# johannes-graeter/limo

Measured on AMD Instinct MI355X. Metric: keyframe-BA window solves/sec (5 KF, ~2k landmarks), higher is better.
Workload: dtype f64; 1 GPU; C2: KITTI-00-shaped windows, 5 keyframes x 2000 landmarks, LiDAR depth + ground plane, solveTrimmed schedule {2, trim 5%, <=100 LM iterations}; batch_windows_per_gpu=16384, distinct_windows_per_gpu=4096, observations_per_batch=144288124, depth_observations_per_batch=68405568, parallelism=single, converged=16328

## Files before the change

### limo_amd/csrc/kba_items.hpp

```cpp
#pragma once
#include "kba_layout.hpp"
#include "kba_lm.hpp"
#include "kba_math.hpp"

#ifndef KBA_SYNC
#define KBA_SYNC() ((void)0)
#endif
#if defined(KBA_PROFILE_TICKS) && defined(__HIPCC__)
__device__ long long kba_ticks[2][24];
#endif
#if defined(KBA_PROFILE_TICKS) && defined(__HIP_DEVICE_COMPILE__)
#define KBA_TICK(n)                                                                   \
    do {                                                                              \
        if (w == 0 && (tid == 0 || tid == nt - 1)) kba_ticks[tid != 0][n] = clock64(); \
    } while (0)
#else
#define KBA_TICK(n) ((void)0)
#endif

namespace kba {

struct LinLane {
    double e[kLinPartial];
    int fail;
// ... 310 lines not shown
    const WinDesc& wd = bv.win[w];
    part[0] = part[1] = part[5] = 0.0;
    for (int j = 0; j < wd.n_view; ++j) {
        cam[j].fail = 0;
        for (int i = 0; i < kLinPartial; ++i) cam[j].e[i] = 0.0;
    }
    const int state = bv.lm_state[gl];
    if (state == 0) return 0;
    LmAcc acc;
    for (int i = 0; i < 6; ++i) acc.V[i] = 0.0;
    for (int i = 0; i < 3; ++i) acc.g[i] = 0.0;
    int fail = 0;
    for (int j = 0; j < wd.n_view; ++j) {
        const int s = bv.lm_slot[(int64_t)j * bv.SL + gl];
        if (s < 0) continue;
        LinIn in;
        lin_fetch(bv, s, gl, in);
        const double* vl = bv.view_lin + (int64_t)kViewLin * (wd.view0 + j);
        double r3[3], c4[4];
        if (j < wd.n_view_fixed0) {
            if (!lin_obs<false>(vl, c, in, want_cost, r3, c4, cam[j])) fail = 1;
        } else {
            if (!lin_obs<true>(vl, c, in, want_cost, r3, c4, cam[j])) fail = 1;
        }
        bv.obs_c[s] = c4[0];
        bv.obs_c[bv.SO + s] = c4[3];
        lin_lm_accum(vl, r3, c4, acc);
    }
    if (state == 1) {
        LmTailIn t;
        lin_lm_tail_fetch(bv, w, gl, t);
        lin_lm_finish(bv, c, gl, bv.lm + 3 * (int64_t)gl, t, acc, part);
    }
    return fail;
}

KBA_HD void trim_residual_lane(const BatchView& bv, int b, int t, double* plane_rep, double* plane_dep) {
    if (t >= bv.blk_n[b]) return;
    const int view = bv.blk_view[b];
    const int64_t o = bv.blk_obs0[b] + t;
    const int gl = bv.obs_lm[o];
    double nr = -1.0, nd = -1.0;
    if (bv.lm_state[gl]) {
        const double* cam = bv.view_cam + 16 * (int64_t)view;
        double ruv[2], rd, zc[3];
        if (obs_residual(bv.pose + 7 * (int64_t)bv.view_kf[view], cam + 4, cam + 13, cam[0], cam[1], cam[2],
                         bv.lm + 3 * (int64_t)gl, bv.obs_u[o], bv.obs_v[o], bv.obs_d[o], ruv, &rd, zc)) {
            nr = sqrt(ruv[0] * ruv[0] + ruv[1] * ruv[1]);
        } else {
// ... 178 lines not shown
    while ((ca + 1) * lda - (ca + 1) * ca / 2 <= i) ++ca;
    cb = ca + (i - (ca * lda - ca * (ca - 1) / 2));
}
KBA_HD int schur_col(int i, int nfq);
KBA_HD int64_t schur_need_offset(int ca, int cb, int nf, int nfq, int nfp) {
    if (cb < nf) return (int64_t)schur_col(ca, nfq) * nfp + schur_col(cb, nfq);
    const int za = schur_col(ca, nfq);
    return za < nfq ? (int64_t)za * nfp + nfq : (int64_t)nfq * nfp + za;
}
KBA_HD void slab_reduce_entry(const BatchView& bv, int w, int n_shards, int i) {
    const WinDesc& wd = bv.win[w];
    const int64_t slab = (int64_t)wd.nf_pad * wd.nf_pad;
    int ca, cb;
    schur_need_decode(i, wd.nf, ca, cb);
    const double* sp = bv.S_part + wd.spart_off + schur_need_offset(ca, cb, wd.nf, wd.nfq, wd.nf_pad);
    double a = 0.0;
    const int q0 = (ca >= wd.nfq || (cb >= wd.nfq && cb < wd.nf)) ? wd.n_sblk_plain : 0;
    for (int q = q0; q < wd.n_sblk; ++q) a += sp[q * slab];
    bv.S_red[wd.sred_off / n_shards + i] = a;
}

KBA_HD int schur_col(int i, int nfq) {
    return i + (i >= nfq ? 1 : 0);
}

struct LogProd {
    double m;
    int e;
};
KBA_HD void logprod_mul(LogProd& a, double x) {
    int ex;
    a.m *= frexp(x, &ex);
    a.e += ex;
}
KBA_HD double logprod_log(const LogProd& a) { return log(a.m) + static_cast<double>(a.e) * 0.69314718055994530942; }

KBA_HD void backsub_lane(const BatchView& bv, const SolveConsts& c, int w, int gl, double* part) {
    part[2] = part[3] = part[4] = part[6] = part[7] = 0.0;
    const int state = bv.lm_state[gl];
    const double* xp = bv.lm + 3 * (int64_t)gl;
    const double x[3] = {xp[0], xp[1], xp[2]};
    double xc[3] = {x[0], x[1], x[2]};
    if (state == 0) {
        double* o = bv.lm_c + 3 * (int64_t)gl;
        o[0] = xc[0];
        o[1] = xc[1];
// ... 671 lines not shown
    const int nc = wd.nc, nf = wd.nf, nfp = wd.nf_pad, lda = nf + 1;
    double* A = scratch;
    double* y = A + nf * lda;
    double* dl = y + nf;
    int* fl = reinterpret_cast<int*>(dl + nc);
    double* red = dl + nc + (nf + 1) / 2 + 1;
    double* Hs = red + coop_red_doubles(3, nt);
    const double radius = bv.st[w].radius;
    const double* Hg = bv.Hcc + wd.hcc_off;
    const double* sc = bv.scale_c + wd.cam0;
    const int32_t* cs = bv.cslot + wd.cam0;
    double* yc = bv.yc + wd.cam0;
    double* dc = bv.delta_c + wd.cam0;
    const int slab = c.schur_packed ? schur_need_pad(nf) : nfp * nfp;
    const int nfq = wd.nfq;
    KBA_TICK(8);
    for (int a = tid; a < nc; a += nt)
        if (cs[a] >= 0) fl[cs[a]] = a;
    KBA_SYNC();
    const double* sp = c.schur_nslab > 0 ? bv.S_red + wd.sred_off : bv.S_part + wd.spart_off;
    const int n_need = nf * (nf + 1) / 2 + nf;
    const int n_slab = c.schur_nslab > 0 ? c.schur_nslab : schur_slabs(wd, c.schur_span, c.schur_span_gp);
    const int q_gp = c.schur_nslab > 0 ? 0 : (schur_plain_slabs(wd, c.schur_span) & ~3);
    constexpr int kE = 4;
    for (int i0 = tid; i0 < n_need; i0 += kE * nt) {
        double s[kE], acc[kE][4];
        int64_t off[kE];
        int dst[kE], qs[kE];
        for (int e = 0; e < kE; ++e) {
            const int i = i0 + e * nt;
            dst[e] = -1;
            off[e] = 0;
            qs[e] = n_slab;
            s[e] = 0.0;
            for (int r = 0; r < 4; ++r) acc[e][r] = 0.0;
            if (i >= n_need) continue;
            int ca, cb;
            schur_need_decode(i, nf, ca, cb);
            const int a = fl[ca];
            if (cb < nf) {
                const int b = fl[cb];
                double v = sc[a] * sc[b] * Hg[a * nc + b];
                Hs[i] = v;
                if (ca == cb) v += fmin(fmax(v, c.min_lm_diagonal), c.max_lm_diagonal) / radius;
                s[e] = v;
            } else {
                s[e] = sc[a] * bv.gc[wd.cam0 + a];
                Hs[i] = s[e];
            }
            off[e] = c.schur_packed ? (int64_t)i : schur_need_offset(ca, cb, nf, nfq, nfp);
            dst[e] = ca * lda + cb;
            qs[e] = (ca >= nfq || (cb >= nfq && cb < nf)) ? q_gp : 0;
        }
        int q = 0;
        for (; q + 4 <= n_slab; q += 4)
            for (int e = 0; e < kE; ++e)
                for (int r = 0; r < 4; ++r) {
                    const bool on = q >= qs[e];
                    const double v = sp[(int64_t)(on ? q + r : n_slab - 1) * slab + off[e]];
                    acc[e][r] += on ? v : 0.0;
                }
        for (; q < n_slab; ++q)
            for (int e = 0; e < kE; ++e) {
                const bool on = q >= qs[e];
                const double v = sp[(int64_t)(on ? q : n_slab - 1) * slab + off[e]];
                acc[e][0] += on ? v : 0.0;
            }
        for (int e = 0; e < kE; ++e)
            if (dst[e] >= 0) A[dst[e]] = s[e] - ((acc[e][0] + acc[e][1]) + (acc[e][2] + acc[e][3]));
    }
    KBA_SYNC();
    KBA_TICK(9);
    bool failed = false;
    (void)flag;
    const int tw = nt >= 16 ? 16 : 1, th = nt / tw, tx = tid % tw;
    const int ty = nt == 256 ? ((tid >> 4) & 3) * 4 + (tid >> 6) : tid / tw;
#if defined(__HIP_DEVICE_COMPILE__)
    if (nt == 256) {
        typedef double v4d_t __attribute__((ext_vector_type(4)));
        const int lane = tid & 63, wave = tid >> 6, li = lane & 15, kq = lane >> 4;
        double* invd = y;
        if (tid == 0) *flag = 0;
        KBA_SYNC();
        for (int kb = 0; kb < nf; kb += 4) {
            const int kbe = kb + 4 < nf ? kb + 4 : nf;
            if (wave == 0 && nf < 64) {
                auto bcast = [](double v, int from) {
                    return __hiloint2double(__builtin_amdgcn_readlane(__double2hiint(v), from), __builtin_amdgcn_readlane(__double2loint(v), from));
                };
                double rw[4];
#pragma unroll
                for (int q = 0; q < 4; ++q) rw[q] = (kb + q < kbe && lane <= nf) ? A[(kb + q) * lda + lane] : 0.0;
// ... 433 lines not shown
```

### limo_amd/csrc/kba_kernels.hip

```cpp
#include <hip/hip_runtime.h>

#include <type_traits>

#define KBA_SYNC() __syncthreads()
#include "kba_items.hpp"

namespace kba {

__device__ __forceinline__ double wave_sum(double v) {
#pragma unroll
    for (int off = 32; off > 0; off >>= 1) v += __shfl_down(v, off, 64);
    return v;
}
__device__ __forceinline__ double wave_max(double v) {
#pragma unroll
    for (int off = 32; off > 0; off >>= 1) v = fmax(v, __shfl_down(v, off, 64));
    return v;
}

template <int N>
__device__ __forceinline__ void block_sum(const double* vals, double* lds , double* out_global) {
    const int lane = threadIdx.x & 63, wave = threadIdx.x >> 6;
#pragma unroll
    for (int i = 0; i < N; ++i) {
// ... 347 lines not shown
        d_n = bv.obs_d[o];
    }
    const int rs14_idx = rs14_index(lane);
    const int j_cam0 = wd.n_view_fixed0;
    for (int j = 0; j < j_cam0; ++j) {
        VT vl = vc + (int64_t)j * kVStride;
        const int s = s_cur;
        in.u = u_n;
        in.v = v_n;
        in.d = d_n;
        s_cur = s_nxt;
        s_nxt = j + 2 < n_view ? slot[(int64_t)(j + 2) * bv.SL] : -1;
        {
            const int64_t o = s_cur >= 0 ? s_cur : 0;
            u_n = bv.obs_u[o];
            v_n = bv.obs_v[o];
            d_n = bv.obs_d[o];
        }
        const bool have = state != 0 && s >= 0;
        in.live = have;
        LinLane l;
        double r3[3], c4[4];
        if (!lin_obs<false>(vl, c, in, want_cost, r3, c4, l)) fail = 1;
        {
            const int64_t o = have ? s : dump;
            bv.obs_c[o] = c4[0];
            bv.obs_c[bv.SO + o] = c4[3];
        }
        accum(vl, r3, c4);
        const double tot = wave_sum_all(l.e[0]);
        if (lane < kLinPartial) lv_lds[(j * kLinWaves + wave) * kLinPartial + lane] = lane == 0 ? tot : 0.0;
    }
    for (int j = j_cam0; j < n_view; ++j) {
        VT vl = vc + (int64_t)j * kVStride;
        const int s = s_cur;
        in.u = u_n;
        in.v = v_n;
        in.d = d_n;
        s_cur = s_nxt;
        s_nxt = j + 2 < n_view ? slot[(int64_t)(j + 2) * bv.SL] : -1;
        {
            const int64_t o = s_cur >= 0 ? s_cur : 0;
            u_n = bv.obs_u[o];
            v_n = bv.obs_v[o];
            d_n = bv.obs_d[o];
        }
        const bool have = state != 0 && s >= 0;
        in.live = have;
        LinLane l;
        double r3[3], c4[4];
        if (!lin_obs_core(vl, c, in, want_cost, r3, c4, l.e[0])) fail = 1;
// ... 229 lines not shown
        }
    }
}

constexpr int kSpBatch = 4;
constexpr int kSpKf = 72;

__host__ __device__ inline int schur_lean_ld(int ncol) { return ncol | 1; }
__host__ __device__ inline int schur_lean_lds_bytes(int ncol) {
    return (3 * kSchurLm * schur_lean_ld(ncol) + 16 + 4 * kSpKf) * (int)sizeof(double) + 4 * 12 * (int)sizeof(int);
}

template <bool COOP>
__device__ __forceinline__ void schur_wave_sync() {
    if constexpr (COOP) {
        __builtin_amdgcn_fence(__ATOMIC_RELEASE, "workgroup");
        __builtin_amdgcn_wave_barrier();
        __builtin_amdgcn_fence(__ATOMIC_ACQUIRE, "workgroup");
    } else {
        __syncthreads();
    }
}
template <int TM, bool GP, bool COOP>
__device__ __forceinline__ void schur_lean_group(const BatchView& bv, int sb, int span, int span_gp, double* smem) {
    const int w = bv.sblk_win[sb];
    if (!COOP && !bv.st[w].active) return;
    const WinDesc& wd = bv.win[w];
    const int nfq = wd.nfq, nfp = wd.nf_pad;
    const int ncol = GP ? wd.nf + 1 : nfq + 1;
    const int ld = schur_lean_ld(ncol);
    const int Tt = (ncol + 15) / 16;
    constexpr bool kTT = !GP && TM == 2;
    const bool two_tile = kTT && Tt == 2;
    double* Z = smem;
    double* kc = Z + 3 * kSchurLm * ld + 16;
    int* zcs = reinterpret_cast<int*>(kc + 4 * kSpKf);
    const int lane = COOP ? (int)(threadIdx.x & 63) : (int)threadIdx.x, li = lane & 15, kq = lane >> 4;
    const int n_fk = wd.n_fk;
    int my_view = -1, my_kl = -1;
    if (kq < n_fk) {
        my_kl = wd.fk[kq];
        my_view = wd.fk_view[kq];
        double* mine = kc + kq * kSpKf;
        const double* pose = bv.pose + 7 * (int64_t)(wd.kf0 + my_kl);
        if (li == 0) {
            double R[9];
            quat_R(pose, R);
// ... 193 lines not shown
        } else {
            if constexpr (TM >= 3) {
#pragma unroll
                for (int h = 0; h < 12; h += 2) {
                    double pn[2][3];
#pragma unroll
                    for (int j = 0; j < 2; ++j)
#pragma unroll
                        for (int t = 0; t < 3; ++t) pn[j][t] = zp[(h + j) * 4 * ld + 16 * t];
#pragma unroll
                    for (int j = 0; j < 2; ++j) {
                        acc[0] = __builtin_amdgcn_mfma_f64_16x16x4f64(pn[j][0], pn[j][0], acc[0], 0, 0, 0);
                        acc[1] = __builtin_amdgcn_mfma_f64_16x16x4f64(pn[j][0], pn[j][1], acc[1], 0, 0, 0);
                        acc[2] = __builtin_amdgcn_mfma_f64_16x16x4f64(pn[j][0], pn[j][2], acc[2], 0, 0, 0);
                        acc[3] = __builtin_amdgcn_mfma_f64_16x16x4f64(pn[j][1], pn[j][1], acc[3], 0, 0, 0);
                        acc[4] = __builtin_amdgcn_mfma_f64_16x16x4f64(pn[j][1], pn[j][2], acc[4], 0, 0, 0);
                        acc[5] = __builtin_amdgcn_mfma_f64_16x16x4f64(pn[j][2], pn[j][2], acc[5], 0, 0, 0);
                    }
                }
            }
        }
        schur_wave_sync<COOP>();
    }
    double* out = bv.S_part + wd.spart_off + (int64_t)schur_slab_of(wd, sb, span, span_gp) * ((int64_t)nfp * nfp);
    const int T = nfp / 16;
    if (two_tile) {
        double* St = Z;
        for (int i = lane; i < 1024; i += 64) St[i] = 0.0;
        schur_wave_sync<COOP>();
#pragma unroll
        for (int r = 0; r < 4; ++r) {
            const int row = kq + 4 * r;
            {
                const int col = 8 + li;
                if (row <= col && col < nfq) St[row * 32 + col] = acc[0][r];
            }
            {
                const int a = row < 8 ? row : row + 8, b = mq;
                if (a <= b && b < nfq && !(a < 8 && b >= 16)) St[a * 32 + b] = acc[1][r];
            }
        }
        if (have) {
#pragma unroll
            for (int a = 0; a < 6; ++a) {
                double v = yt[a];
                v += __shfl_xor(v, 1, 64);
                v += __shfl_xor(v, 2, 64);
                v += __shfl_xor(v, 4, 64);
                v += __shfl_xor(v, 8, 64);
                if (li == 0) St[(zcs[kq * 12] + a) * 32 + nfq] = v;
            }
        }
        schur_wave_sync<COOP>();
        for (int tc = 0; tc < (T < 2 ? T : 2); ++tc)
            for (int tr = 0; tr <= tc; ++tr) {
#pragma unroll
                for (int r = 0; r < 4; ++r) {
                    const int row = tr * 16 + kq + 4 * r, col = tc * 16 + li;
                    out[row * nfp + col] = St[row * 32 + col];
                }
            }
        return;
    }
    if constexpr (kTT) {
#pragma unroll
        for (int r = 0; r < 4; ++r) {
            const int row = kq + 4 * r, col = li;
            out[row * nfp + col] = (row < ncol && col < ncol) ? acc[0][r] : 0.0;
        }
    } else {
        int idx = 0;
#pragma unroll
        for (int tr = 0; tr < TM; ++tr)
#pragma unroll
            for (int tc = tr; tc < TM; ++tc) {
                if (tc < T) {
#pragma unroll
                    for (int r = 0; r < 4; ++r) {
                        const int row = tr * 16 + kq + 4 * r, col = tc * 16 + li;
                        out[row * nfp + col] = (row < ncol && col < ncol) ? acc[idx][r] : 0.0;
                    }
                }
                ++idx;
            }
        if constexpr (GP) {
            for (int tc = TM; tc < T; ++tc)
                for (int tr = 0; tr <= tc; ++tr) {
#pragma unroll
                    for (int r = 0; r < 4; ++r) out[(tr * 16 + kq + 4 * r) * nfp + tc * 16 + li] = 0.0;
                }
        }
    }
}
template <int TM, bool GP, int WAVES>
__global__ __launch_bounds__(64) __attribute__((amdgpu_waves_per_eu(WAVES, WAVES))) void k_schur_lean(
    BatchView bv, const int32_t* wl, int span, int span_gp) {
    const int sb = wl_at(bv, wl, blockIdx.x);
    if (sb < 0) return;
    extern __shared__ __attribute__((aligned(16))) double smem[];
    schur_lean_group<TM, GP, false>(bv, sb, span, span_gp, smem);
}

template <int TMP, int TMG>
__global__ __launch_bounds__(64) void k_schur_lean_pair(BatchView bv, const int32_t* wl_plain, int n_plain_cap, const int32_t* wl_gp, int span, int span_gp) {
    extern __shared__ __attribute__((aligned(16))) double smem[];
    if ((int)blockIdx.x < n_plain_cap) {
        const int sb = wl_at(bv, wl_plain, blockIdx.x);
        if (sb >= 0) schur_lean_group<TMP, false, false>(bv, sb, span, span_gp, smem);
    } else {
        const int sb = wl_at(bv, wl_gp, blockIdx.x - n_plain_cap);
        if (sb >= 0) schur_lean_group<TMG, true, false>(bv, sb, span, span_gp, smem);
    }
}

__global__ __launch_bounds__(kBlock) __attribute__((amdgpu_waves_per_eu(3, 3))) void k_cam_assemble(BatchView bv, SolveConsts c, const int32_t* wl) {
    const int w = wl_at(bv, wl, blockIdx.x);
    if (w < 0) return;
    WinState& st = bv.st[w];
    extern __shared__ __attribute__((aligned(16))) double smem[];
    if (st.active && st.need_lin) {
        const int64_t so = bv.win[w].cam_scr_off;
        if (so >= 0)
            cam_assemble(bv, c, w, threadIdx.x, blockDim.x, bv.cam_scratch + so);
        else
            cam_assemble(bv, c, w, threadIdx.x, blockDim.x, smem);
        __syncthreads();
#ifdef KBA_PROFILE_TICKS
        if (w == 0 && threadIdx.x == 0)
            for (int l = 0; l < 2; ++l)
                printf("[ticks cam_assemble %s lane] observation blocks %lld, ground-plane rows %lld, regulariser rows %lld, their sums %lld, mask + store %lld, reductions %lld\n",
                       l ? "last" : "first", kba_ticks[l][1] - kba_ticks[l][0], kba_ticks[l][2] - kba_ticks[l][1], kba_ticks[l][3] - kba_ticks[l][2],
                       kba_ticks[l][4] - kba_ticks[l][3], kba_ticks[l][5] - kba_ticks[l][4], kba_ticks[l][6] - kba_ticks[l][5]);
#endif
        if (threadIdx.x == 0) lm_decide_lin(st, bv.red[w], bv.reg_cost[2 * w + 1], c);
// ... 468 lines not shown
    do {                                    \
        const long long n_ = wall_clock64(); \
        tk[i] += n_ - tl;                   \
        tl = n_;                            \
    } while (0)
#else
#define KBA_CTICK(i)
#endif
#define KBA_GSYNC()                                        \
    do {                                                   \
        if (!coop_sync(bar, bar + 2, G, gen, a.abort_host, a.timeout_ticks)) return; \
    } while (0)
    const int lb0 = wd.lblk0, lb1 = wd.lblk0 + wd.n_lblk;
    const int n_pg = (wd.n_sblk_plain + c.schur_span - 1) / c.schur_span;
    const int n_gg = (wd.n_sblk - wd.n_sblk_plain + c.schur_span_gp - 1) / c.schur_span_gp;
    auto schur_phase = [&](int first_worker) __attribute__((always_inline)) {
        if (g < first_worker) return;
        const int n_workers = (G - first_worker) * (kBlock / 64);
        double* mine = smem + (size_t)wave * a.schur_lds;
        for (int t = (g - first_worker) * (kBlock / 64) + wave; t < n_pg + n_gg; t += n_workers) {
            if (t < n_pg) {
                const int sb = wd.sblk0 + t * c.schur_span;
                if (a.vp == 1)
                    schur_lean_group<1, false, true>(bv, sb, c.schur_span, c.schur_span_gp, mine);
                else
                    schur_lean_group<2, false, true>(bv, sb, c.schur_span, c.schur_span_gp, mine);
            } else {
                const int sb = wd.sblk0 + wd.n_sblk_plain + (t - n_pg) * c.schur_span_gp;
                if (a.vg == 1)
                    schur_lean_group<1, true, true>(bv, sb, c.schur_span, c.schur_span_gp, mine);
                else if (a.vg == 2)
                    schur_lean_group<2, true, true>(bv, sb, c.schur_span, c.schur_span_gp, mine);
                else
                    schur_lean_group<3, true, true>(bv, sb, c.schur_span, c.schur_span_gp, mine);
            }
            schur_wave_sync<true>();
        }
    };
    const int n_solves = 2 * c.num_trim_rounds + 1;
    for (int si = 0; si < n_solves; ++si) {
        const bool final_solve = si == n_solves - 1, retry = !final_solve && (si & 1);
        const int max_iter = final_solve ? c.max_iters : (retry ? 3 * c.trim_iters : c.trim_iters);
        KBA_GSYNC();
        if (g == 0) {
            if (tid == 0) {
                bool sel = true;
                if (!final_solve) sel = wd.do_trim != 0;
                if (retry) sel = sel && (st.solve_initial_cost - st.solve_final_cost <= 0.0);
                lm_solve_init(st, sel, max_iter, c);
            }
            __syncthreads();
            if (st.active && st.need_lin && tid < wd.n_view) view_consts_item(bv, wd.view0 + tid);
        }
        KBA_GSYNC();
        const long long t0 = a.cap_ticks > 0 ? (long long)wall_clock64() : 0ll;
        for (;;) {
            double* outr = a.red + (int64_t)w * kCoopRedStride;
// ... 266 lines not shown
```

### limo_amd/csrc/kba_layout.hpp

```cpp
#pragma once
#include <stddef.h>
#include <stdint.h>

#include "../../include/limo_hip.h"

namespace kba {

constexpr int kMaxKf = 20;
constexpr int kMaxViews = 64;
constexpr int kViewLin = 64;
constexpr int kCamSlots = 10;
constexpr int kMaxNc = kMaxKf * kCamSlots;
constexpr int kBlock = 256;
constexpr int kObsPerLane = 4;
constexpr int kObsBlock = kBlock * kObsPerLane;
constexpr int kSchurLm = 16;
constexpr int kSchurLmPerBlock = 64;
constexpr int kMaxRegRows = 1 + (kMaxKf - 1) * 5 + 3 * kMaxKf;

constexpr int kGpRed = 65;
constexpr int kLinPartial = 28;
constexpr int kLinWaves = 4;

struct EvalChunk {
// ... 61 lines not shown
    double step2;
    double cand2;
    double cand_cost;
    int32_t lin_fail, chol_fail, cand_fail, pad;
};

enum SchedPhase { PH_IDLE = 0, PH_TRIM_SOLVE = 1, PH_RETRY = 2, PH_TRIM = 3, PH_FINAL = 4, PH_DONE = 5 };

enum SchedList { SL_LBLK = 0, SL_SPLAIN, SL_SFGP, SL_SGEN, SL_WIN, SL_TBLK, SL_TLBLK, SL_TWIN, SL_COUNT };

struct SolveConsts {
    double a_rep, a_dep;
    double inv_a_rep2, inv_a_dep2;
    double function_tolerance, gradient_tolerance, parameter_tolerance;
    double initial_radius, max_radius, min_radius, min_lm_diagonal, max_lm_diagonal, min_relative_decrease;
    int32_t max_invalid, jacobi_scaling;
    double depth_quantile, reprojection_quantile;
    int32_t min_groups, pad;
    int32_t schur_span;
    int32_t schur_span_gp;
    int32_t num_trim_rounds, trim_iters, max_iters;
    int32_t schur_nslab;
    int32_t schur_packed;
};

struct BatchView {
    int32_t n_win, TK, TL, TO, TV, TG, n_blk, n_lblk, n_sblk, Vmax;
    int64_t SO, SL, SG;
    const WinDesc* win;
    WinState* st;
    WinRed* red;
    double *pose, *pdir, *pdist, *lm;
    double *pose_c, *pdir_c, *pdist_c, *lm_c;
    const int32_t* kf_win;
    const int32_t* kf_blk0;
    const int32_t* kf_nblk;
    const int32_t* kf_gp0;
    const int32_t* kf_ngp;
    uint8_t* cmask;
    uint8_t* cpresent;
    const int32_t* cslot;
    const int32_t* lm_win;
    const int32_t* lm_id;
    const double* lm_weight;
    uint8_t* lm_state;
    const int32_t* lm_gp;
// ... 82 lines not shown
```

### limo_amd/csrc/limo_hip.hip

```cpp
#include <hip/hip_runtime.h>
#include <rccl/rccl.h>

#include <algorithm>
#include <chrono>
#include <cmath>
#include <cstdio>
#include <cstring>
#include <atomic>
#include <string>
#include <thread>
#include <vector>

#include "kba_kernels.hip"

#include "kba_buffers.hpp"
#include "kba_rows.hpp"

using namespace kba;

#include "limo_ctx.hpp"

#define HIP_TRY(ctx, expr)                                                                       \
    do {                                                                                         \
        hipError_t e__ = (expr);                                                                 \
// ... 318 lines not shown
                    nc_lds = std::max(nc_lds, (int)d.nc);
                    nf_lds = std::max(nf_lds, (int)d.nf);
                    nv_lds = std::max(nv_lds, (int)d.n_view);
                }
            asm_bytes = cam_assemble_scratch(nc_lds, kBlock, nv_lds) * (int)sizeof(double);
            solve_bytes = cam_solve_scratch(nc_lds, kBlock, nf_lds) * (int)sizeof(double);
        }
        int max_lm = 1;
        for (const WinDesc& d : P.win) max_lm = std::max(max_lm, (int)d.n_lm);
        {
            int np2 = 1;
            while (np2 < max_lm) np2 <<= 1;
            trim_bytes = np2 <= kTrimMaxSort ? np2 * 12 + max_lm + 16 : 16;
        }
        HIP_TRY(ctx, hipFuncSetAttribute((const void*)k_cam_assemble, hipFuncAttributeMaxDynamicSharedMemorySize, asm_bytes));
        HIP_TRY(ctx, hipFuncSetAttribute((const void*)k_cam_solve, hipFuncAttributeMaxDynamicSharedMemorySize, solve_bytes));
        HIP_TRY(ctx, hipFuncSetAttribute((const void*)k_trim_select, hipFuncAttributeMaxDynamicSharedMemorySize, trim_bytes));
        for (auto& e : act_ev) HIP_TRY(ctx, hipEventCreateWithFlags(&e, hipEventDisableTiming));
        HIP_TRY(ctx, hipEventCreate(&ev_total_a));
        HIP_TRY(ctx, hipEventCreate(&ev_total_b));
        return LIMO_OK;
    }

    bool pristine = true;
    int reset_state() {
        pristine = true;
        HIP_TRY(ctx, hipMemcpyAsync(bv.st, st0.data(), sizeof(WinState) * st0.size(), hipMemcpyHostToDevice, ctx->stream));
        HIP_TRY(ctx, hipMemcpyAsync(bv.pose, d_pose0, sizeof(double) * 7 * P.TK, hipMemcpyDeviceToDevice, ctx->stream));
        HIP_TRY(ctx, hipMemcpyAsync(bv.pdir, d_pdir0, sizeof(double) * 3 * P.TK, hipMemcpyDeviceToDevice, ctx->stream));
        HIP_TRY(ctx, hipMemcpyAsync(bv.pdist, d_pdist0, sizeof(double) * P.TK, hipMemcpyDeviceToDevice, ctx->stream));
        HIP_TRY(ctx, hipMemcpyAsync(bv.lm, d_lm0, sizeof(double) * 3 * P.TL, hipMemcpyDeviceToDevice, ctx->stream));
        HIP_TRY(ctx, hipMemcpyAsync(bv.lm_state, d_lm_state0, P.TL, hipMemcpyDeviceToDevice, ctx->stream));
        return LIMO_OK;
    }

    void note(hipError_t e, const char* what) {
        if (e != hipSuccess && rc == LIMO_OK) {
            rc = LIMO_ERR_RUNTIME;
            ctx->err = std::string(what) + ": " + hipGetErrorString(e);
        }
    }
#define LAUNCH_CHECK(what) note(hipGetLastError(), what)

    void set_span() {
        c.schur_span = shard_P > 1 ? 1 : 2;
        c.schur_span_gp = 1;
        c.schur_nslab = shard_P > 1 ? shard_P : 0;
        c.schur_packed = shard_P > 1 ? 1 : 0;
    }

    const int32_t* list_blk(size_t i) const { return shard_P > 1 ? rl[i].blk : (use_wl ? d_wl_blk : nullptr); }
    const int32_t* list_lblk(size_t i) const { return shard_P > 1 ? rl[i].lblk : (use_wl ? d_wl_lblk : nullptr); }
    const int32_t* list_sblk(size_t i) const { return shard_P > 1 ? rl[i].sblk : d_wl_sblk; }
    int count_blk(size_t i) const { return shard_P > 1 ? rl[i].n_blk : n_wl_blk; }
    int count_lblk(size_t i) const { return shard_P > 1 ? rl[i].n_lblk : n_wl_lblk; }
    int count_sblk(size_t i) const { return shard_P > 1 ? rl[i].n_sblk : n_wl_sblk; }
    int count_sblk_plain(size_t i) const { return shard_P > 1 ? rl[i].n_sblk_plain : n_wl_sblk_plain; }
    int count_sblk_fgp(size_t i) const { return shard_P > 1 ? rl[i].n_sblk_fgp : n_wl_sblk_fgp; }
    int shard_of(size_t i) const { return shard_P > 1 ? local_shards[i] : 0; }

    void exchange(int point) {
        if (shard_P == 1) return;
        hipStream_t s = ctx->stream;
        size_t off, count;
        xl.range(point, off, count);
        for (size_t i = 0; i < pv.size(); ++i) {
            if (shard_virtual) {
                hipLaunchKernelGGL(k_unpack, dim3(cdiv((int64_t)count, 256)), dim3(256), 0, s, xl, (const WinDesc*)d_win_orig, (const double*)(blocks[i] + off), arena_c,
                                   local_shards[i], (int64_t)off, (int64_t)count);
                LAUNCH_CHECK("k_unpack");
            } else {
// ... 239 lines not shown
        if (cur == 0) return P.n_win;
        const int slot = (cur - 1) & 3;
        note(hipEventSynchronize(act_ev[slot]), "sync n_active");
        if (rc != LIMO_OK) return 0;
        const int a = h_active[slot];
        static const bool trace = std::getenv("KBA_TRACE_ACTIVE") != nullptr;
        if (trace) std::fprintf(stderr, "[kba] iteration %d: active %d, listed %d, span %d\n", cur - 1, a, listed, c.schur_span);
        if (a > 0 && listed >= 8 && 2 * a <= listed) rebatch();
        return a;
    }

    void expire(int) override {
        if (assemble_pending) {
            assemble_pending = false;
            exchange(1);
            assemble(it_no - 1);
        }
        hipLaunchKernelGGL(k_expire, dim3(cdiv(P.n_win, 256)), dim3(256), 0, ctx->stream, bv);
        LAUNCH_CHECK("k_expire");
    }

    void step() override {
        hipStream_t s = ctx->stream;
        for (size_t i = 0; i < pv.size(); ++i)
            if (count_lblk(i)) {
                hipLaunchKernelGGL(k_lm_damp, dim3(count_lblk(i)), dim3(kBlock), 0, s, pv[i], c, list_lblk(i));
                LAUNCH_CHECK("k_lm_damp");
            }
        {
            EventPair* ep = timed(LIMO_KERNEL_SCHUR);
            for (size_t i = 0; i < pv.size(); ++i) {
                int n_plain = count_sblk_plain(i), n_fgp = count_sblk_fgp(i);
                const int n_gen = count_sblk(i) - n_plain - n_fgp;
                int span = c.schur_span, span_gp = c.schur_span_gp;
                const int32_t* wlp = list_sblk(i);
                if (n_plain) {
                    void* args[] = {(void*)&pv[i], (void*)&wlp, (void*)&span, (void*)&span_gp};
                    note(hipLaunchKernel(schur_fn_plain, dim3(n_plain), dim3(64), args, plain_lds_bytes, s), "launch k_schur_lean");
                    LAUNCH_CHECK("k_schur_lean");
                    wlp += n_plain;
                }
                if (n_fgp) {
                    void* args[] = {(void*)&pv[i], (void*)&wlp, (void*)&span, (void*)&span_gp};
                    note(hipLaunchKernel(schur_fn_leangp, dim3(n_fgp), dim3(64), args, leangp_lds_bytes, s), "launch k_schur_lean (gp)");
                    LAUNCH_CHECK("k_schur_lean (gp)");
                    wlp += n_fgp;
                }
                if (n_gen) {
                    void* args[] = {(void*)&pv[i], (void*)&wlp, (void*)&span, (void*)&span_gp};
                    note(hipLaunchKernel(schur_fn_gen, dim3(n_gen), dim3(64 * kWideWaves), args, wide_lds_bytes, s), "launch k_schur_wide");
                    LAUNCH_CHECK("k_schur_wide");
                }
            }
            if (ep) note(hipEventRecord(ep->b, s), "hipEventRecord");
        }
        if (shard_P > 1) {
            if (n_wl_win)
                for (size_t i = 0; i < pv.size(); ++i) {
                    const int32_t* wlw = use_wl ? (const int32_t*)d_wl_win : (const int32_t*)nullptr;
                    hipLaunchKernelGGL(k_shard_reduce, dim3(n_wl_win), dim3(kBlock), 0, s, pv[i], wlw, shard_of(i), 1);
                    hipLaunchKernelGGL(k_slab_reduce, dim3(n_wl_win, 8), dim3(kBlock), 0, s, pv[i], wlw, shard_P);
                    LAUNCH_CHECK("k_slab_reduce");
                }
            if (assemble_pending) {
                assemble_pending = false;
                exchange(3);
// ... 147 lines not shown
        for (int k = 0; k < SL_COUNT; ++k) cap[k] = std::min(g.cap[k], bound * g.mx[k]);
        auto L = [&](int k) { return (const int32_t*)(g.d_lists + sv.sched_off[k] + 1); };
        if (round > 0) note(hipStreamWaitEvent(s, g.trim_ev, 0), "wait trim");
        hipLaunchKernelGGL(k_sched_advance, dim3(cdiv(g.n_slots, 256)), dim3(256), 0, s, sv, c);
        hipLaunchKernelGGL(k_sched_scan, dim3(1), dim3(kSchedThreads), 0, s, sv, round);
        hipLaunchKernelGGL(k_sched_fill, dim3(cdiv(g.n_slots, 4)), dim3(256), 0, s, sv, c);
        LAUNCH_CHECK("scheduler kernels");
        note(hipEventRecord(g.sched_ev, s), "record sched");
        note(hipStreamWaitEvent(g.trim_stream, g.sched_ev, 0), "wait sched");
        if (cap[SL_TBLK]) hipLaunchKernelGGL(k_trim_residual, dim3(cap[SL_TBLK]), dim3(kBlock), 0, g.trim_stream, sv, d_plane_rep, d_plane_dep, L(SL_TBLK));
        if (cap[SL_TLBLK]) hipLaunchKernelGGL(k_trim_max, dim3(cap[SL_TLBLK]), dim3(kBlock), 0, g.trim_stream, sv, (const double*)d_plane_rep, (const double*)d_plane_dep, 0, 1);
        hipLaunchKernelGGL(k_trim_select, dim3(cap[SL_TWIN]), dim3(kBlock), trim_bytes, g.trim_stream, sv, c);
        LAUNCH_CHECK("trim kernels");
        note(hipEventRecord(g.trim_ev, g.trim_stream), "record trim");
        {
            EventPair* ep = time_kernels ? timed(LIMO_KERNEL_LINEARIZE, s) : nullptr;
            if (cap[SL_LBLK]) launch_lin_lm(cap[SL_LBLK], s, sv, L(SL_LBLK));
            if (ep) note(hipEventRecord(ep->b, s), "hipEventRecord");
        }
        hipLaunchKernelGGL(k_cam_assemble, dim3(cap[SL_WIN]), dim3(kBlock), asm_bytes, s, sv, c, L(SL_WIN));
        LAUNCH_CHECK("linearisation kernels");
        {
            EventPair* ep = time_kernels ? timed(LIMO_KERNEL_SCHUR, s) : nullptr;
            int span = c.schur_span, span_gp = c.schur_span_gp;
            const bool pair = schur_pair_ok && bound <= kSchurPairBound && cap[SL_SPLAIN] && cap[SL_SFGP];
            if (pair) {
                const int32_t *wlp = L(SL_SPLAIN), *wlg = L(SL_SFGP);
                int n_plain_cap = cap[SL_SPLAIN];
                void* args[] = {(void*)&sv, (void*)&wlp, (void*)&n_plain_cap, (void*)&wlg, (void*)&span, (void*)&span_gp};
                note(hipLaunchKernel((const void*)k_schur_lean_pair<2, 3>, dim3(cap[SL_SPLAIN] + cap[SL_SFGP]), dim3(64), args, std::max(plain_lds_bytes, leangp_lds_bytes), s),
                     "launch k_schur_lean_pair");
            }
            if (!pair && cap[SL_SPLAIN]) {
                const int32_t* wlp = L(SL_SPLAIN);
                void* args[] = {(void*)&sv, (void*)&wlp, (void*)&span, (void*)&span_gp};
                note(hipLaunchKernel(schur_fn_plain, dim3(cap[SL_SPLAIN]), dim3(64), args, plain_lds_bytes, s), "launch k_schur_lean");
            }
            if (!pair && cap[SL_SFGP]) {
                const int32_t* wlp = L(SL_SFGP);
                void* args[] = {(void*)&sv, (void*)&wlp, (void*)&span, (void*)&span_gp};
                note(hipLaunchKernel(schur_fn_leangp, dim3(cap[SL_SFGP]), dim3(64), args, leangp_lds_bytes, s), "launch k_schur_lean (gp)");
            }
            if (cap[SL_SGEN]) {
                const int32_t* wlp = L(SL_SGEN);
                void* args[] = {(void*)&sv, (void*)&wlp, (void*)&span, (void*)&span_gp};
                note(hipLaunchKernel(schur_fn_gen, dim3(cap[SL_SGEN]), dim3(64 * kWideWaves), args, wide_lds_bytes, s), "launch k_schur_wide");
            }
            if (ep) note(hipEventRecord(ep->b, s), "hipEventRecord");
        }
        hipLaunchKernelGGL(k_cam_solve, dim3(cap[SL_WIN]), dim3(kBlock), solve_bytes, s, sv, c, L(SL_WIN));
        if (cap[SL_LBLK]) hipLaunchKernelGGL(k_backsub, dim3(cap[SL_LBLK]), dim3(kBlock), 0, s, sv, c, L(SL_LBLK));
        hipLaunchKernelGGL(k_step_decide, dim3(cap[SL_WIN]), dim3(64), 0, s, sv, c, L(SL_WIN));
        if (cap[SL_LBLK])
            hipLaunchKernelGGL(k_after_step, dim3(cap[SL_LBLK]), dim3(kBlock), 0, s, sv, c, L(SL_LBLK));
        LAUNCH_CHECK("step kernels");
        note(hipEventRecord(g.round_ev[round & 3], s), "record round");
    }

    static constexpr int kWgMaxLblk = 8;
    bool wg_solve_applies() const {
        if (shard_P != 1 || P.evaluate_only || P.n_sblk != 0 || P.n_win < 1) return false;
        if (const char* e = std::getenv("KBA_NO_WG_SOLVE"))
            if (std::atoi(e) != 0) return false;
// ... 28 lines not shown
        int G = 1;
        for (const WinDesc& d : P.win) {
            if (!d.schur_fast || d.cam_scr_off >= 0 || d.nf_pad * d.nf_pad > kCoopRedStride) return false;
            const int tasks = (d.n_sblk_plain + c.schur_span - 1) / c.schur_span + (d.n_sblk - d.n_sblk_plain + c.schur_span_gp - 1) / c.schur_span_gp;
            G = std::max(G, std::max((int)d.n_lblk, tasks ? 1 + (tasks + kBlock / 64 - 1) / (kBlock / 64) : 1));
        }
        G = std::min(G, 32);
        if (P.n_win > kCoopMaxWg || coop_lds_bytes() > kCamLdsCapBytes) return false;
        const int per8 = ((int)P.n_win + 7) / 8;
        coop_xcd = 8 * per8 > kCoopMaxWg ? 0 : 1;
        G = std::max(1, std::min(G, coop_xcd ? kCoopMaxWg / (8 * per8) : kCoopMaxWg / (int)P.n_win));
        coop_G = G;
        return true;
    }
    bool solve_coop() {
        const int lds = coop_lds_bytes();
        if (!d_coop_bar && dmalloc((void**)&d_coop_bar, sizeof(int32_t) * 8 * P.n_win)) return false;
        if (!d_coop_red && dmalloc((void**)&d_coop_red, sizeof(double) * kCoopRedStride * P.n_win)) return false;
        if (hipFuncSetAttribute((const void*)k_solve_coop, hipFuncAttributeMaxDynamicSharedMemorySize, lds) != hipSuccess) {
            (void)hipGetLastError();
            return false;
        }
        note(hipMemsetAsync(d_coop_bar, 0, sizeof(int32_t) * 8 * P.n_win, ctx->stream), "memset barrier words");
        h_active[8] = 0;
        CoopParams cp;
        cp.G = coop_G;
        cp.xcd_map = coop_xcd;
        const int coop_grid = coop_xcd ? 8 * coop_G * (((int)P.n_win + 7) / 8) : (int)P.n_win * coop_G;
        cp.vp = schur_vp;
        cp.vg = schur_vg;
        cp.schur_lds = (std::max(plain_lds_bytes, leangp_lds_bytes) + 15) / 16 * 16 / (int)sizeof(double);
        cp.cap_ticks = opts.max_solver_time_sec > 0.0 ? std::max(1ll, (long long)(opts.max_solver_time_sec * 1e8)) : 0ll;
        cp.timeout_ticks = 5000000ll;
        if (const char* e = std::getenv("KBA_COOP_TIMEOUT_MS")) cp.timeout_ticks = std::max(0ll, (long long)(std::atof(e) * 1e5));
        cp.bar = d_coop_bar;
        cp.abort_host = d_h_active + 8;
        cp.plane_rep = d_plane_rep;
        cp.plane_dep = d_plane_dep;
        cp.red = d_coop_red;
        void* args[] = {(void*)&bv, (void*)&c, (void*)&cp};
        int per_cu = 0, n_cu = 0;
        if (hipOccupancyMaxActiveBlocksPerMultiprocessor(&per_cu, (const void*)k_solve_coop, kBlock, (size_t)lds) != hipSuccess ||
            hipDeviceGetAttribute(&n_cu, hipDeviceAttributeMultiprocessorCount, ctx->device) != hipSuccess || per_cu * n_cu < coop_grid) {
            (void)hipGetLastError();
            return false;
        }
        if (hipLaunchKernel((const void*)k_solve_coop, dim3(coop_grid), dim3(kBlock), args, lds, ctx->stream) != hipSuccess) {
            (void)hipGetLastError();
            return false;
        }
        coop_launched = true;
        return true;
    }

    int solve_streaming() {
        int n_groups = stream_slots() >= 4096 ? 3 : P.n_win >= 512 ? 2 : 1;
        if (const char* e = std::getenv("KBA_GROUPS")) n_groups = std::max(1, std::min(4, std::atoi(e)));
        if (stream_setup(n_groups) != LIMO_OK) return LIMO_ERR_RUNTIME;
        set_span();
        hipStream_t s0 = ctx->stream;
        groups[0].stream = s0;
        HIP_TRY(ctx, hipMemsetAsync(d_sched_ctl, 0, sizeof(int32_t) * 8, s0));
        for (StreamGroup& g : groups) {
            HIP_TRY(ctx, hipMemsetAsync(g.d_slot_win, 0xFF, sizeof(int32_t) * std::max(1, g.n_slots), s0));
            for (int i = 0; i < 4; ++i) g.h_done[i] = 0;
        }
        HIP_TRY(ctx, hipEventRecord(start_ev, s0));
        for (size_t gi = 1; gi < groups.size(); ++gi) HIP_TRY(ctx, hipStreamWaitEvent(groups[gi].stream, start_ev, 0));
        const bool time_kernels = groups.size() == 1;
        constexpr int kLag = 2;
        static const bool sched_trace = std::getenv("KBA_SCHED_TRACE") != nullptr;
        std::vector<int> done_curve;
        double enq_us = 0.0;
        const auto t_solve0 = std::chrono::steady_clock::now();
        bool finished = false;
        int done_seen = 0;
        for (int round = 0; !finished; ++round) {
            const int in_flight_max = (int)P.n_win - done_seen;
            const auto t_enq0 = std::chrono::steady_clock::now();
            for (StreamGroup& g : groups) enqueue_round(g, round, time_kernels, in_flight_max);
            if (sched_trace) enq_us += std::chrono::duration<double, std::micro>(std::chrono::steady_clock::now() - t_enq0).count();
            if (rc != LIMO_OK) break;
// ... 715 lines not shown
```

Measured before the change: 36690 windows/s.

## Pack Schur partial slabs as upper-triangle need lists and drop redundant obs_c stores

The lean Schur kernels now write per-slab partial Schur complements in a packed upper-triangular layout. Plain slabs are sized to nfq and ground-plane slabs to nf, instead of full nfp×nfp padded squares with zero fills. The reduction inside the camera solve reads through matching packed offsets, and the coop path clears S_part when it reuses the buffer. Separately, obs_c stores are dropped for fixed views in the landmark lane and removed from the linearisation kernel. This is meant to cut global write and read traffic on the slabs, in exchange for extra index arithmetic and a risk that fixed-view costs are no longer stored if any consumer needs them.

```diff
diff --git a/limo_amd/csrc/kba_items.hpp b/limo_amd/csrc/kba_items.hpp
--- a/limo_amd/csrc/kba_items.hpp
+++ b/limo_amd/csrc/kba_items.hpp
@@ -356,9 +356,9 @@
             if (!lin_obs<false>(vl, c, in, want_cost, r3, c4, cam[j])) fail = 1;
         } else {
             if (!lin_obs<true>(vl, c, in, want_cost, r3, c4, cam[j])) fail = 1;
-        }
-        bv.obs_c[s] = c4[0];
-        bv.obs_c[bv.SO + s] = c4[3];
+            bv.obs_c[s] = c4[0];
+            bv.obs_c[bv.SO + s] = c4[3];
+        }
         lin_lm_accum(vl, r3, c4, acc);
     }
     if (state == 1) {
@@ -583,6 +583,23 @@
 
 KBA_HD int schur_col(int i, int nfq) {
     return i + (i >= nfq ? 1 : 0);
+}
+
+KBA_HD int schur_need_index(int n, int ca, int cb) { return ca * (n + 1) - ca * (ca - 1) / 2 + (cb - ca); }
+KBA_HD int64_t slab_packed_base(int q, int n_plain, int nf, int nfq) {
+    return q < n_plain ? (int64_t)q * schur_need_pad(nfq) : (int64_t)n_plain * schur_need_pad(nfq) + (int64_t)(q - n_plain) * schur_need_pad(nf);
+}
+KBA_HD int slab_packed_read(bool gp, int ca, int cb, int nf, int nfq) {
+    if (gp) return schur_need_index(nf, ca, cb);
+    if (ca >= nfq || (cb >= nfq && cb < nf)) return -1;
+    return schur_need_index(nfq, ca, cb < nf ? cb : nfq);
+}
+KBA_HD int slab_packed_write(bool gp, int zr, int zc, int nf, int nfq) {
+    const int n = gp ? nf : nfq;
+    if (zr > zc || zc > n || (zr == nfq && zc == nfq)) return -1;
+    if (zc == nfq) return schur_need_index(n, zr, n);
+    if (zr == nfq) return schur_need_index(n, zc - 1, n);
+    return schur_need_index(n, zr - (zr > nfq ? 1 : 0), zc - (zc > nfq ? 1 : 0));
 }
 
 struct LogProd {
@@ -1300,52 +1317,65 @@
     const int n_need = nf * (nf + 1) / 2 + nf;
     const int n_slab = c.schur_nslab > 0 ? c.schur_nslab : schur_slabs(wd, c.schur_span, c.schur_span_gp);
     const int q_gp = c.schur_nslab > 0 ? 0 : (schur_plain_slabs(wd, c.schur_span) & ~3);
+    const bool pk = c.slab_packed && wd.schur_fast && c.schur_nslab == 0;
+    const int n_pk = pk ? schur_plain_slabs(wd, c.schur_span) : 0;
+    const int64_t stride_pl = pk ? schur_need_pad(nfq) : 0, stride_gp = pk ? schur_need_pad(nf) : slab;
+    const int64_t skip_base = pk ? (n_slab > n_pk ? slab_packed_base(n_slab - 1, n_pk, nf, nfq) : 0) : (int64_t)(n_slab - 1) * slab;
     constexpr int kE = 4;
     for (int i0 = tid; i0 < n_need; i0 += kE * nt) {
-        double s[kE], acc[kE][4];
-        int64_t off[kE];
+        double acc[kE][4];
+        int off[kE], off_pl[kE];
         int dst[kE], qs[kE];
         for (int e = 0; e < kE; ++e) {
             const int i = i0 + e * nt;
             dst[e] = -1;
             off[e] = 0;
+            off_pl[e] = -1;
             qs[e] = n_slab;
-            s[e] = 0.0;
             for (int r = 0; r < 4; ++r) acc[e][r] = 0.0;
             if (i >= n_need) continue;
             int ca, cb;
             schur_need_decode(i, nf, ca, cb);
             const int a = fl[ca];
+            double s_e;
             if (cb < nf) {
                 const int b = fl[cb];
                 double v = sc[a] * sc[b] * Hg[a * nc + b];
                 Hs[i] = v;
                 if (ca == cb) v += fmin(fmax(v, c.min_lm_diagonal), c.max_lm_diagonal) / radius;
-                s[e] = v;
+                s_e = v;
             } else {
-                s[e] = sc[a] * bv.gc[wd.cam0 + a];
-                Hs[i] = s[e];
+                s_e = sc[a] * bv.gc[wd.cam0 + a];
+                Hs[i] = s_e;
             }
-            off[e] = c.schur_packed ? (int64_t)i : schur_need_offset(ca, cb, nf, nfq, nfp);
+            off[e] = (c.schur_packed || pk) ? i : (int)schur_need_offset(ca, cb, nf, nfq, nfp);
+            if (pk) off_pl[e] = slab_packed_read(false, ca, cb, nf, nfq);
             dst[e] = ca * lda + cb;
+            A[dst[e]] = s_e;
             qs[e] = (ca >= nfq || (cb >= nfq && cb < nf)) ? q_gp : 0;
         }
         int q = 0;
         for (; q + 4 <= n_slab; q += 4)
             for (int e = 0; e < kE; ++e)
                 for (int r = 0; r < 4; ++r) {
-                    const bool on = q >= qs[e];
-                    const double v = sp[(int64_t)(on ? q + r : n_slab - 1) * slab + off[e]];
+                    const bool plain = q + r < n_pk;
+                    const int64_t base = plain ? (int64_t)(q + r) * stride_pl : n_pk * stride_pl + (int64_t)(q + r - n_pk) * stride_gp;
+                    const int o = plain ? off_pl[e] : off[e];
+                    const bool on = q >= qs[e] && o >= 0;
+                    const double v = sp[on ? base + o : skip_base + off[e]];
                     acc[e][r] += on ? v : 0.0;
                 }
         for (; q < n_slab; ++q)
             for (int e = 0; e < kE; ++e) {
-                const bool on = q >= qs[e];
-                const double v = sp[(int64_t)(on ? q : n_slab - 1) * slab + off[e]];
+                const bool plain = q < n_pk;
+                const int64_t base = plain ? (int64_t)q * stride_pl : n_pk * stride_pl + (int64_t)(q - n_pk) * stride_gp;
+                const int o = plain ? off_pl[e] : off[e];
+                const bool on = q >= qs[e] && o >= 0;
+                const double v = sp[on ? base + o : skip_base + off[e]];
                 acc[e][0] += on ? v : 0.0;
             }
         for (int e = 0; e < kE; ++e)
-            if (dst[e] >= 0) A[dst[e]] = s[e] - ((acc[e][0] + acc[e][1]) + (acc[e][2] + acc[e][3]));
+            if (dst[e] >= 0) A[dst[e]] = A[dst[e]] - ((acc[e][0] + acc[e][1]) + (acc[e][2] + acc[e][3]));
     }
     KBA_SYNC();
     KBA_TICK(9);
diff --git a/limo_amd/csrc/kba_kernels.hip b/limo_amd/csrc/kba_kernels.hip
--- a/limo_amd/csrc/kba_kernels.hip
+++ b/limo_amd/csrc/kba_kernels.hip
@@ -393,11 +393,6 @@
         LinLane l;
         double r3[3], c4[4];
         if (!lin_obs<false>(vl, c, in, want_cost, r3, c4, l)) fail = 1;
-        {
-            const int64_t o = have ? s : dump;
-            bv.obs_c[o] = c4[0];
-            bv.obs_c[bv.SO + o] = c4[3];
-        }
         accum(vl, r3, c4);
         const double tot = wave_sum_all(l.e[0]);
         if (lane < kLinPartial) lv_lds[(j * kLinWaves + wave) * kLinPartial + lane] = lane == 0 ? tot : 0.0;
@@ -673,7 +668,7 @@
     }
 }
 template <int TM, bool GP, bool COOP>
-__device__ __forceinline__ void schur_lean_group(const BatchView& bv, int sb, int span, int span_gp, double* smem) {
+__device__ __forceinline__ void schur_lean_group(const BatchView& bv, int sb, int span, int span_gp, int slab_packed, double* smem) {
     const int w = bv.sblk_win[sb];
     if (!COOP && !bv.st[w].active) return;
     const WinDesc& wd = bv.win[w];
@@ -913,8 +908,37 @@
         }
         schur_wave_sync<COOP>();
     }
-    double* out = bv.S_part + wd.spart_off + (int64_t)schur_slab_of(wd, sb, span, span_gp) * ((int64_t)nfp * nfp);
+    const bool packed = !COOP && slab_packed != 0;
+    const int q_slab = schur_slab_of(wd, sb, span, span_gp);
+    double* out = bv.S_part + wd.spart_off +
+                  (packed ? slab_packed_base(q_slab, schur_plain_slabs(wd, span), wd.nf, nfq) : (int64_t)q_slab * ((int64_t)nfp * nfp));
     const int T = nfp / 16;
+    if (two_tile && packed) {
+#pragma unroll
+        for (int r = 0; r < 4; ++r) {
+            const int row = kq + 4 * r;
+            {
+                const int col = 8 + li;
+                if (row <= col && col < nfq) out[slab_packed_write(false, row, col, wd.nf, nfq)] = acc[0][r];
+            }
+            {
+                const int a = row < 8 ? row : row + 8, b = mq;
+                if (a <= b && b < nfq && !(a < 8 && b >= 16)) out[slab_packed_write(false, a, b, wd.nf, nfq)] = acc[1][r];
+            }
+        }
+        if (have) {
+#pragma unroll
+            for (int a = 0; a < 6; ++a) {
+                double v = yt[a];
+                v += __shfl_xor(v, 1, 64);
+                v += __shfl_xor(v, 2, 64);
+                v += __shfl_xor(v, 4, 64);
+                v += __shfl_xor(v, 8, 64);
+                if (li == 0) out[slab_packed_write(false, zcs[kq * 12] + a, nfq, wd.nf, nfq)] = v;
+            }
+        }
+        return;
+    }
     if (two_tile) {
         double* St = Z;
         for (int i = lane; i < 1024; i += 64) St[i] = 0.0;
@@ -957,7 +981,12 @@
 #pragma unroll
         for (int r = 0; r < 4; ++r) {
             const int row = kq + 4 * r, col = li;
-            out[row * nfp + col] = (row < ncol && col < ncol) ? acc[0][r] : 0.0;
+            if (packed) {
+                const int k = slab_packed_write(false, row, col, wd.nf, nfq);
+                if (k >= 0) out[k] = acc[0][r];
+            } else {
+                out[row * nfp + col] = (row < ncol && col < ncol) ? acc[0][r] : 0.0;
+            }
         }
     } else {
         int idx = 0;
@@ -969,38 +998,44 @@
 #pragma unroll
                     for (int r = 0; r < 4; ++r) {
                         const int row = tr * 16 + kq + 4 * r, col = tc * 16 + li;
-                        out[row * nfp + col] = (row < ncol && col < ncol) ? acc[idx][r] : 0.0;
+                        if (packed) {
+                            const int k = slab_packed_write(GP, row, col, wd.nf, nfq);
+                            if (k >= 0) out[k] = acc[idx][r];
+                        } else {
+                            out[row * nfp + col] = (row < ncol && col < ncol) ? acc[idx][r] : 0.0;
+                        }
                     }
                 }
                 ++idx;
             }
         if constexpr (GP) {
-            for (int tc = TM; tc < T; ++tc)
-                for (int tr = 0; tr <= tc; ++tr) {
-#pragma unroll
-                    for (int r = 0; r < 4; ++r) out[(tr * 16 + kq + 4 * r) * nfp + tc * 16 + li] = 0.0;
-                }
+            if (!packed)
+                for (int tc = TM; tc < T; ++tc)
+                    for (int tr = 0; tr <= tc; ++tr) {
+#pragma unroll
+                        for (int r = 0; r < 4; ++r) out[(tr * 16 + kq + 4 * r) * nfp + tc * 16 + li] = 0.0;
+                    }
         }
     }
 }
 template <int TM, bool GP, int WAVES>
 __global__ __launch_bounds__(64) __attribute__((amdgpu_waves_per_eu(WAVES, WAVES))) void k_schur_lean(
-    BatchView bv, const int32_t* wl, int span, int span_gp) {
+    BatchView bv, const int32_t* wl, int span, int span_gp, int slab_packed) {
     const int sb = wl_at(bv, wl, blockIdx.x);
     if (sb < 0) return;
     extern __shared__ __attribute__((aligned(16))) double smem[];
-    schur_lean_group<TM, GP, false>(bv, sb, span, span_gp, smem);
+    schur_lean_group<TM, GP, false>(bv, sb, span, span_gp, slab_packed, smem);
 }
 
 template <int TMP, int TMG>
-__global__ __launch_bounds__(64) void k_schur_lean_pair(BatchView bv, const int32_t* wl_plain, int n_plain_cap, const int32_t* wl_gp, int span, int span_gp) {
+__global__ __launch_bounds__(64) void k_schur_lean_pair(BatchView bv, const int32_t* wl_plain, int n_plain_cap, const int32_t* wl_gp, int span, int span_gp, int slab_packed) {
     extern __shared__ __attribute__((aligned(16))) double smem[];
     if ((int)blockIdx.x < n_plain_cap) {
         const int sb = wl_at(bv, wl_plain, blockIdx.x);
-        if (sb >= 0) schur_lean_group<TMP, false, false>(bv, sb, span, span_gp, smem);
+        if (sb >= 0) schur_lean_group<TMP, false, false>(bv, sb, span, span_gp, slab_packed, smem);
     } else {
         const int sb = wl_at(bv, wl_gp, blockIdx.x - n_plain_cap);
-        if (sb >= 0) schur_lean_group<TMG, true, false>(bv, sb, span, span_gp, smem);
+        if (sb >= 0) schur_lean_group<TMG, true, false>(bv, sb, span, span_gp, slab_packed, smem);
     }
 }
 
@@ -1515,17 +1550,17 @@
             if (t < n_pg) {
                 const int sb = wd.sblk0 + t * c.schur_span;
                 if (a.vp == 1)
-                    schur_lean_group<1, false, true>(bv, sb, c.schur_span, c.schur_span_gp, mine);
+                    schur_lean_group<1, false, true>(bv, sb, c.schur_span, c.schur_span_gp, 0, mine);
                 else
-                    schur_lean_group<2, false, true>(bv, sb, c.schur_span, c.schur_span_gp, mine);
+                    schur_lean_group<2, false, true>(bv, sb, c.schur_span, c.schur_span_gp, 0, mine);
             } else {
                 const int sb = wd.sblk0 + wd.n_sblk_plain + (t - n_pg) * c.schur_span_gp;
                 if (a.vg == 1)
-                    schur_lean_group<1, true, true>(bv, sb, c.schur_span, c.schur_span_gp, mine);
+                    schur_lean_group<1, true, true>(bv, sb, c.schur_span, c.schur_span_gp, 0, mine);
                 else if (a.vg == 2)
-                    schur_lean_group<2, true, true>(bv, sb, c.schur_span, c.schur_span_gp, mine);
+                    schur_lean_group<2, true, true>(bv, sb, c.schur_span, c.schur_span_gp, 0, mine);
                 else
-                    schur_lean_group<3, true, true>(bv, sb, c.schur_span, c.schur_span_gp, mine);
+                    schur_lean_group<3, true, true>(bv, sb, c.schur_span, c.schur_span_gp, 0, mine);
             }
             schur_wave_sync<true>();
         }
diff --git a/limo_amd/csrc/kba_layout.hpp b/limo_amd/csrc/kba_layout.hpp
--- a/limo_amd/csrc/kba_layout.hpp
+++ b/limo_amd/csrc/kba_layout.hpp
@@ -107,6 +107,7 @@
     int32_t num_trim_rounds, trim_iters, max_iters;
     int32_t schur_nslab;
     int32_t schur_packed;
+    int32_t slab_packed;
 };
 
 struct BatchView {
diff --git a/limo_amd/csrc/limo_hip.hip b/limo_amd/csrc/limo_hip.hip
--- a/limo_amd/csrc/limo_hip.hip
+++ b/limo_amd/csrc/limo_hip.hip
@@ -364,6 +364,7 @@
         return LIMO_OK;
     }
 
+    bool spart_has_packed = false;
     bool pristine = true;
     int reset_state() {
         pristine = true;
@@ -389,6 +390,7 @@
         c.schur_span_gp = 1;
         c.schur_nslab = shard_P > 1 ? shard_P : 0;
         c.schur_packed = shard_P > 1 ? 1 : 0;
+        c.slab_packed = shard_P > 1 ? 0 : 1;
     }
 
     const int32_t* list_blk(size_t i) const { return shard_P > 1 ? rl[i].blk : (use_wl ? d_wl_blk : nullptr); }
@@ -674,6 +676,7 @@
 
     void step() override {
         hipStream_t s = ctx->stream;
+        if (c.slab_packed) spart_has_packed = true;
         for (size_t i = 0; i < pv.size(); ++i)
             if (count_lblk(i)) {
                 hipLaunchKernelGGL(k_lm_damp, dim3(count_lblk(i)), dim3(kBlock), 0, s, pv[i], c, list_lblk(i));
@@ -684,16 +687,16 @@
             for (size_t i = 0; i < pv.size(); ++i) {
                 int n_plain = count_sblk_plain(i), n_fgp = count_sblk_fgp(i);
                 const int n_gen = count_sblk(i) - n_plain - n_fgp;
-                int span = c.schur_span, span_gp = c.schur_span_gp;
+                int span = c.schur_span, span_gp = c.schur_span_gp, packed = c.slab_packed;
                 const int32_t* wlp = list_sblk(i);
                 if (n_plain) {
-                    void* args[] = {(void*)&pv[i], (void*)&wlp, (void*)&span, (void*)&span_gp};
+                    void* args[] = {(void*)&pv[i], (void*)&wlp, (void*)&span, (void*)&span_gp, (void*)&packed};
                     note(hipLaunchKernel(schur_fn_plain, dim3(n_plain), dim3(64), args, plain_lds_bytes, s), "launch k_schur_lean");
                     LAUNCH_CHECK("k_schur_lean");
                     wlp += n_plain;
                 }
                 if (n_fgp) {
-                    void* args[] = {(void*)&pv[i], (void*)&wlp, (void*)&span, (void*)&span_gp};
+                    void* args[] = {(void*)&pv[i], (void*)&wlp, (void*)&span, (void*)&span_gp, (void*)&packed};
                     note(hipLaunchKernel(schur_fn_leangp, dim3(n_fgp), dim3(64), args, leangp_lds_bytes, s), "launch k_schur_lean (gp)");
                     LAUNCH_CHECK("k_schur_lean (gp)");
                     wlp += n_fgp;
@@ -887,23 +890,23 @@
         LAUNCH_CHECK("linearisation kernels");
         {
             EventPair* ep = time_kernels ? timed(LIMO_KERNEL_SCHUR, s) : nullptr;
-            int span = c.schur_span, span_gp = c.schur_span_gp;
+            int span = c.schur_span, span_gp = c.schur_span_gp, packed = c.slab_packed;
             const bool pair = schur_pair_ok && bound <= kSchurPairBound && cap[SL_SPLAIN] && cap[SL_SFGP];
             if (pair) {
                 const int32_t *wlp = L(SL_SPLAIN), *wlg = L(SL_SFGP);
                 int n_plain_cap = cap[SL_SPLAIN];
-                void* args[] = {(void*)&sv, (void*)&wlp, (void*)&n_plain_cap, (void*)&wlg, (void*)&span, (void*)&span_gp};
+                void* args[] = {(void*)&sv, (void*)&wlp, (void*)&n_plain_cap, (void*)&wlg, (void*)&span, (void*)&span_gp, (void*)&packed};
                 note(hipLaunchKernel((const void*)k_schur_lean_pair<2, 3>, dim3(cap[SL_SPLAIN] + cap[SL_SFGP]), dim3(64), args, std::max(plain_lds_bytes, leangp_lds_bytes), s),
                      "launch k_schur_lean_pair");
             }
             if (!pair && cap[SL_SPLAIN]) {
                 const int32_t* wlp = L(SL_SPLAIN);
-                void* args[] = {(void*)&sv, (void*)&wlp, (void*)&span, (void*)&span_gp};
+                void* args[] = {(void*)&sv, (void*)&wlp, (void*)&span, (void*)&span_gp, (void*)&packed};
                 note(hipLaunchKernel(schur_fn_plain, dim3(cap[SL_SPLAIN]), dim3(64), args, plain_lds_bytes, s), "launch k_schur_lean");
             }
             if (!pair && cap[SL_SFGP]) {
                 const int32_t* wlp = L(SL_SFGP);
-                void* args[] = {(void*)&sv, (void*)&wlp, (void*)&span, (void*)&span_gp};
+                void* args[] = {(void*)&sv, (void*)&wlp, (void*)&span, (void*)&span_gp, (void*)&packed};
                 note(hipLaunchKernel(schur_fn_leangp, dim3(cap[SL_SFGP]), dim3(64), args, leangp_lds_bytes, s), "launch k_schur_lean (gp)");
             }
             if (cap[SL_SGEN]) {
@@ -978,6 +981,10 @@
             return false;
         }
         note(hipMemsetAsync(d_coop_bar, 0, sizeof(int32_t) * 8 * P.n_win, ctx->stream), "memset barrier words");
+        if (spart_has_packed) {
+            note(hipMemsetAsync(bv.S_part, 0, sizeof(double) * (size_t)std::max<int64_t>(1, P.spart_total), ctx->stream), "clear packed Schur slabs");
+            spart_has_packed = false;
+        }
         h_active[8] = 0;
         CoopParams cp;
         cp.G = coop_G;
@@ -994,7 +1001,9 @@
         cp.plane_rep = d_plane_rep;
         cp.plane_dep = d_plane_dep;
         cp.red = d_coop_red;
-        void* args[] = {(void*)&bv, (void*)&c, (void*)&cp};
+        SolveConsts cc = c;
+        cc.slab_packed = 0;
+        void* args[] = {(void*)&bv, (void*)&cc, (void*)&cp};
         int per_cu = 0, n_cu = 0;
         if (hipOccupancyMaxActiveBlocksPerMultiprocessor(&per_cu, (const void*)k_solve_coop, kBlock, (size_t)lds) != hipSuccess ||
             hipDeviceGetAttribute(&n_cu, hipDeviceAttributeMultiprocessorCount, ctx->device) != hipSuccess || per_cu * n_cu < coop_grid) {
@@ -1014,6 +1023,7 @@
         if (const char* e = std::getenv("KBA_GROUPS")) n_groups = std::max(1, std::min(4, std::atoi(e)));
         if (stream_setup(n_groups) != LIMO_OK) return LIMO_ERR_RUNTIME;
         set_span();
+        if (c.slab_packed) spart_has_packed = true;
         hipStream_t s0 = ctx->stream;
         groups[0].stream = s0;
         HIP_TRY(ctx, hipMemsetAsync(d_sched_ctl, 0, sizeof(int32_t) * 8, s0));
```

Result: faster. 37070 windows/s (median of 6 runs) (+1.0%).
